# seorim0/DNN-based-Speech-Enhancement-in-the-frequency-domain

Measured on AMD Instinct MI355X. Metric: train utts/sec (3s@16kHz) DCCRN, higher is better.
Workload: dtype bf16; 1 GPU; DCCRN mask C, SI-SNR, fwd+bwd+Adam, B=32/GPU x 3s@16kHz clips (BASELINE configs[1]); global_batch=32, parallelism=dp1, bn=per-rank statistics, collective=none

## Files before the change

dnn-based-speech-enhancement-in-the-frequency-domain_amd/build.py:

```python
import os
import subprocess
from concurrent.futures import ThreadPoolExecutor

HERE = os.path.dirname(os.path.abspath(__file__))
CSRC = os.path.join(HERE, "csrc")
OBJ = os.path.join(CSRC, "_obj")
LIB = os.path.join(HERE, "libsefd_hip.so")
SOURCES = ["api.hip", "kernels.hip", "rungemm.hip", "rungemm_persist.hip", "cgemm256.hip", "enc0.hip", "lstm_bf16.hip", "lstm_cluster.hip", "lstm_rows.hip", "bn.hip", "cbn.hip", "lms.hip", "pmsqe.hip", "mix.hip", "composite.hip", "fsn.hip", "basemodel.hip", "stft_fft.hip", "thin.hip", "thin_mask.hip", "thin_stage.hip", "layout.hip", "optim.hip", "plan.cpp", "plan_dccrn.cpp", "plan_crn.cpp",
           "plan_fsn.cpp", "plan_seq.cpp", "plan_clstm.cpp", "plan_frontend.cpp", "plan_layers.cpp", "tuning.cpp"]


def _headers():
    hs = [os.path.join(CSRC, f) for f in os.listdir(CSRC) if f.endswith(".h")]
    hs.append(os.path.join(HERE, "..", "include", "sefd.h"))
    return [h for h in hs if os.path.exists(h)]


def _stale(target, deps):
    if not os.path.exists(target):
        return True
    t = os.path.getmtime(target)
    return any(os.path.getmtime(d) > t for d in deps)


def source_digest(paths, extra="") -> str:
    import hashlib
    h = hashlib.sha256(extra.encode())
    for p in sorted(paths):
        h.update(os.path.basename(p).encode())
        with open(p, "rb") as f:
            h.update(f.read())
    return h.hexdigest()


def stamp_current(lib, digest) -> bool:
    try:
        return os.path.exists(lib) and open(lib + ".stamp").read().strip() == digest
    except OSError:
        return False


def write_stamp(lib, digest):
    with open(lib + ".stamp", "w") as f:
        f.write(digest + "\n")


FLAGS = ["--offload-arch=gfx950", "-O3", "-std=c++17", "-fPIC"]


def _digest():
    return source_digest([os.path.join(CSRC, s) for s in SOURCES] + _headers(), " ".join(FLAGS + SOURCES))


def needs_build() -> bool:
    return not stamp_current(LIB, _digest())


def build(force: bool = False, verbose: bool = False) -> str:
    if not force and not needs_build():
        return LIB
    os.makedirs(OBJ, exist_ok=True)
    import fcntl
    with open(os.path.join(OBJ, ".build.lock"), "w") as lock:
        fcntl.flock(lock, fcntl.LOCK_EX)
        try:
            if not force and not needs_build():
                return LIB
            return _build_locked(force, verbose)
        finally:
            fcntl.flock(lock, fcntl.LOCK_UN)


def _build_locked(force, verbose) -> str:
    hipcc = os.environ.get("HIPCC", "/opt/rocm/bin/hipcc")
    heads = _headers()
    jobs = []
    for s in SOURCES:
        src, obj = os.path.join(CSRC, s), os.path.join(OBJ, s + ".o")
        if force or _stale(obj, [src] + heads):
            jobs.append([hipcc] + FLAGS + ["-c", "-o", obj, src])

    def run(cmd):
        if verbose:
            print(" ".join(cmd))
        subprocess.run(cmd, check=True, cwd=CSRC)

    with ThreadPoolExecutor(max_workers=int(os.environ.get("SEFD_BUILD_JOBS", "6"))) as ex:
        list(ex.map(run, jobs))
    run([hipcc, "--offload-arch=gfx950", "-fPIC", "-shared", "-o", LIB] + [os.path.join(OBJ, s + ".o") for s in SOURCES])
    write_stamp(LIB, _digest())
    return LIB


if __name__ == "__main__":
    print(build(force=True, verbose=True))
```

dnn-based-speech-enhancement-in-the-frequency-domain_amd/csrc/dev_common.h:

```cpp
#pragma once
#include <hip/hip_runtime.h>
#include "sefd_desc.h"

namespace sefd {

typedef __attribute__((ext_vector_type(4))) float f32x4;
typedef __attribute__((ext_vector_type(16))) float f32x16;
typedef __attribute__((ext_vector_type(8))) __bf16 bf16x8;

struct bf16_t { uint16_t v; };

struct ArenaBases { char* p[A_COUNT]; int* status; int* dstatus; };
__device__ __forceinline__ void set_status(int* host_word, int* dev_word) {
  if (host_word) __hip_atomic_store(host_word, 1, __ATOMIC_RELAXED, __HIP_MEMORY_SCOPE_SYSTEM);
  if (dev_word) __hip_atomic_store(dev_word, 1, __ATOMIC_RELAXED, __HIP_MEMORY_SCOPE_AGENT);
}

__host__ __device__ __forceinline__ char* rp(const ArenaBases& ab, const Ptr& q) { return ab.p[q.arena] + q.off; }

__device__ __forceinline__ uint32_t pack_bf16x2(float lo, float hi) {
  uint32_t r;
  asm("v_cvt_pk_bf16_f32 %0, %1, %2" : "=v"(r) : "v"(lo), "v"(hi));
  return r;
}
__device__ __forceinline__ uint16_t f2bf(float f) { return (uint16_t)pack_bf16x2(f, 0.f); }

struct QuadT {
  uint32_t sel;
  bool hi2;
  __device__ __forceinline__ explicit QuadT(int lane) : sel((lane & 1) ? 0x03020706u : 0x05040100u), hi2((lane & 2) != 0) {}
  __device__ __forceinline__ uint2 pack(uint32_t p01, uint32_t p23) const {
    const uint32_t n01 = (uint32_t)__builtin_amdgcn_mov_dpp((int)p01, 0xB1, 0xF, 0xF, true);
    const uint32_t n23 = (uint32_t)__builtin_amdgcn_mov_dpp((int)p23, 0xB1, 0xF, 0xF, true);
    const uint32_t q0 = __builtin_amdgcn_perm(n01, p01, sel);
    const uint32_t q1 = __builtin_amdgcn_perm(n23, p23, sel);
    const uint32_t send = hi2 ? q0 : q1, keep = hi2 ? q1 : q0;
    const uint32_t recv = (uint32_t)__builtin_amdgcn_mov_dpp((int)send, 0x4E, 0xF, 0xF, true);
    return make_uint2(hi2 ? recv : keep, hi2 ? keep : recv);
  }
  __device__ __forceinline__ uint2 pack(float v0, float v1, float v2, float v3) const { return pack(pack_bf16x2(v0, v1), pack_bf16x2(v2, v3)); }
};
__device__ __forceinline__ uint32_t xor4(uint32_t x, bool hi4) {
  const uint32_t up = (uint32_t)__builtin_amdgcn_update_dpp(0, (int)x, 0x104, 0xF, 0xF, true);
  const uint32_t dn = (uint32_t)__builtin_amdgcn_update_dpp(0, (int)x, 0x114, 0xF, 0xF, true);
  return hi4 ? dn : up;
}
struct OctW {
  bool hi4;
  __device__ __forceinline__ explicit OctW(int lane) : hi4((lane & 4) != 0) {}
  __device__ __forceinline__ void widen(const uint2 (&pk)[4], uint4 (&out)[2]) const {
#pragma unroll
    for (int h = 0; h < 2; ++h) {
      const uint2 keep = hi4 ? pk[2 * h + 1] : pk[2 * h], send = hi4 ? pk[2 * h] : pk[2 * h + 1];
      const uint2 recv = make_uint2(xor4(send.x, hi4), xor4(send.y, hi4));
      out[h] = hi4 ? make_uint4(recv.x, recv.y, keep.x, keep.y) : make_uint4(keep.x, keep.y, recv.x, recv.y);
    }
  }
};
__device__ __forceinline__ float bf2f(uint16_t h) { return __builtin_bit_cast(float, (uint32_t)h << 16); }

template <int DT> struct Elem;
__device__ __forceinline__ float ld_elem(const char* base, int dt, int64_t i) {
  return dt == DT_BF16 ? bf2f(reinterpret_cast<const uint16_t*>(base)[i]) : reinterpret_cast<const float*>(base)[i];
}
__device__ __forceinline__ void st_elem(char* base, int dt, int64_t i, float v) {
  if (dt == DT_BF16) reinterpret_cast<uint16_t*>(base)[i] = f2bf(v);
  else reinterpret_cast<float*>(base)[i] = v;
}

__device__ __forceinline__ float4 ld4(const char* base, int dt, int64_t i) {
  if (dt == DT_BF16) {
    const uint2 r = *reinterpret_cast<const uint2*>(base + i * 2);
    return make_float4(bf2f(r.x & 0xffff), bf2f(r.x >> 16), bf2f(r.y & 0xffff), bf2f(r.y >> 16));
  }
  return *reinterpret_cast<const float4*>(base + i * 4);
}
__device__ __forceinline__ void st4(char* base, int dt, int64_t i, float4 v) {
  if (dt == DT_BF16) {
    uint2 r;
    r.x = pack_bf16x2(v.x, v.y);
    r.y = pack_bf16x2(v.z, v.w);
    *reinterpret_cast<uint2*>(base + i * 2) = r;
  } else {
    *reinterpret_cast<float4*>(base + i * 4) = v;
  }
}

__device__ __forceinline__ void lds_barrier() {
  asm volatile("s_waitcnt lgkmcnt(0)\n\ts_barrier" ::: "memory");
}

__device__ __forceinline__ void dma16(const void* gsrc, uint32_t lds_wave_base) {
  asm volatile("s_mov_b32 m0, %0\n\ts_nop 0\n\tglobal_load_lds_dwordx4 %1, off" ::"s"(__builtin_amdgcn_readfirstlane(lds_wave_base)), "v"(gsrc)
               : "memory");
}
template <int N>
__device__ __forceinline__ void wait_vm() {
  asm volatile("s_waitcnt vmcnt(%0)" ::"n"(N) : "memory");
}
template <int NL, int S>
__device__ __forceinline__ void wait_stage(int rem) {
  if constexpr (S >= 4) { if (rem >= 2) { wait_vm<2 * NL>(); return; } }
  if constexpr (S >= 3) { if (rem >= 1) { wait_vm<NL>(); return; } }
  wait_vm<0>();
}
__device__ __forceinline__ uint32_t lds_addr(const void* p) {
  return (uint32_t)(uintptr_t)(__attribute__((address_space(3))) const void*)p;
}

__device__ __forceinline__ float wave_sum(float v) {
#pragma unroll
  for (int o = 32; o > 0; o >>= 1) v += __shfl_xor(v, o);
  return v;
}

__device__ __forceinline__ float sigmoidf_(float x) { return __builtin_amdgcn_rcpf(1.f + __expf(-x)); }
__device__ __forceinline__ float tanhf_(float x) { return 1.f - 2.f * __builtin_amdgcn_rcpf(__expf(2.f * x) + 1.f); }

__device__ __forceinline__ uint32_t mix32(uint32_t a, uint32_t b, uint32_t c) {
  uint32_t x = a * 0x9E3779B1u ^ (b + 0x7F4A7C15u) * 0x85EBCA77u ^ (c + 0x632BE5ABu) * 0xC2B2AE3Du;
  x ^= x >> 16; x *= 0x7FEB352Du; x ^= x >> 15; x *= 0x846CA68Bu; x ^= x >> 16;
  return x;
}
__device__ __forceinline__ float drop_scale(uint32_t seed0, uint32_t seed1, int layer, float keep, int64_t i) {
  if (keep >= 1.f) return 1.f;
  const uint32_t r = mix32(seed0 + (uint32_t)layer * 0x51ED27u, seed1 ^ (uint32_t)(i >> 32), (uint32_t)i);
  return ((r >> 8) * (1.f / 16777216.f)) < keep ? 1.f / keep : 0.f;
}

struct BnbCol { float mean, invstd, gamma, beta; };
__device__ __forceinline__ BnbCol bnb_col(const RunGemm& d, const ArenaBases& ab, int n) {
  BnbCol c{0.f, 0.f, 0.f, 0.f};
  if (n < d.N) {
    const float* mi = reinterpret_cast<const float*>(rp(ab, d.bnb_mi));
    c.mean = mi[n]; c.invstd = mi[d.N + n];
    c.gamma = reinterpret_cast<const float*>(rp(ab, d.bnb_gamma))[n];
    c.beta = reinterpret_cast<const float*>(rp(ab, d.bnb_beta))[n];
  }
  return c;
}
__device__ __forceinline__ void bnb_accum(const BnbCol& c, float slope, float dz, float yf, float& s0, float& s1, float& s2) {
  const float xh = (yf - c.mean) * c.invstd;
  const float bn = c.gamma * xh + c.beta;
  const float dbn = bn > 0.f ? dz : slope * dz;
  s0 += dbn;
  s1 += dbn * xh;
  s2 += bn > 0.f ? 0.f : bn * dz;
}

struct StreamKey {
  int dev; hipStream_t st;
  bool operator==(const StreamKey& o) const { return dev == o.dev && st == o.st; }
};
struct StreamKeyHash { size_t operator()(const StreamKey& k) const { return (size_t)(uintptr_t)k.st * 31u + (size_t)k.dev; } };
inline StreamKey stream_key(hipStream_t st) { int dev = 0; (void)hipGetDevice(&dev); return StreamKey{dev, st}; }

void launch_rungemm(const RunGemm& d, const ArenaBases& ab, hipStream_t st);
void launch_wgrad(const RunGemm& d, const ArenaBases& ab, hipStream_t st);
bool launch_cgemm256(const RunGemm& d, const ArenaBases& ab, hipStream_t st);
bool launch_enc0_fwd(const RunGemm& d, const ArenaBases& ab, hipStream_t st);
bool launch_enc0_wgrad(const RunGemm& d, const ArenaBases& ab, hipStream_t st);
bool launch_rundirect(const RunGemm& d, const ArenaBases& ab, hipStream_t st);
bool rundirect_takes(const RunGemm& d);
bool launch_rungemm_persist(const RunGemm& d, const ArenaBases& ab, hipStream_t st);
int rungemm_persist_grid(const RunGemm& d);
bool launch_thin_mask(const RunGemm& d, const ArenaBases& ab, hipStream_t st);
int thin_mask_grid(const RunGemm& d);
bool launch_thin_stage(const RunGemm& d, const ArenaBases& ab, hipStream_t st);
int thin_stage_grid(const RunGemm& d);
enum RunFamily : int { kFamNone = 0, kFamEnc0 = 1, kFamCgemm256 = 2, kFamDirect = 3, kFamTiled = 4, kFamPersist = 5, kFamThinMask = 6, kFamThinStage = 7 };
int rungemm_family(const RunGemm& d);
enum WgradFamily : int { kWgFamNone = 0, kWgFamEnc0 = 1, kWgFamEnc0Fused = 2, kWgFamRank = 3, kWgFamWide256 = 4, kWgFamWide256Ones = 5, kWgFamWide128 = 6,
                         kWgFamDma128 = 7, kWgFamDma64 = 8, kWgFamDma32 = 9, kWgFamBf16_128 = 10, kWgFamBf16_64 = 11, kWgFamF32 = 12 };
int wgrad_family(const RunGemm& d);
void launch_misc(const Op& op, const ArenaBases& ab, hipStream_t st);
void launch_stft_fft(const StftFft& d, const ArenaBases& ab, hipStream_t st);
void launch_istft_fft(const IstftFft& d, const ArenaBases& ab, hipStream_t st);
void launch_ifft_ola(const IfftOla& d, const ArenaBases& ab, hipStream_t st);
void launch_specconv(const SpecConv& d, const ArenaBases& ab, hipStream_t st);
void launch_ola_fold(const Ola& d, const ArenaBases& ab, hipStream_t st);
void launch_specout_adj(const SpecOut& d, const ArenaBases& ab, hipStream_t st);
void launch_nchw_cl(const NchwCl& d, const ArenaBases& ab, hipStream_t st);
void launch_fsn(const Op& op, const ArenaBases& ab, hipStream_t st);
void launch_bn(const Op& op, const ArenaBases& ab, hipStream_t st);
void launch_cbn(const Op& op, const ArenaBases& ab, hipStream_t st);
void launch_lstm_bf16(const LstmRec& d, const ArenaBases& ab, hipStream_t st, bool fwd);
inline int lstm_rev_groups(const LstmRec& d) { return d.rev_mask & ((1 << (d.G < 4 ? d.G : 4)) - 1); }
void launch_lstm_cluster(const LstmRec& d, const ArenaBases& ab, hipStream_t st, bool fwd);
void launch_lstm_rows(const LstmRec& d, const ArenaBases& ab, hipStream_t st, bool fwd);
bool launch_lstm_rows_pair(const LstmRec& d0, const LstmRec& d1, const ArenaBases& ab, hipStream_t st);

}
```

dnn-based-speech-enhancement-in-the-frequency-domain_amd/csrc/rungemm.hip:

```cpp
#include <hip/hip_runtime.h>
#include <cstdlib>
#include "sefd_desc.h"
#include "tuning.h"
#include "dev_common.h"

namespace sefd {

template <typename TA>
struct RowInfo {
  int64_t base0, base1;
  int32_t u, fo;
  bool valid;
};

template <typename TA>
__device__ __forceinline__ uint4 load_a_chunk(const RunGemm& d, const TA* x0, const TA* x1, const Seg& sg,
                                              int64_t base0, int64_t base1, int u, int fo, bool rvalid, int j0) {
  constexpr int VEC = 16 / sizeof(TA);
  uint4 z = make_uint4(0, 0, 0, 0);
  if (!rvalid) return z;
  if (sg.src < 0) {
    if (j0 == 0) {
      if (sizeof(TA) == 4) z.x = 0x3f800000u; else z.x = 0x3f80u;
    }
// ... 1053 lines not shown
#pragma unroll
    for (int e = 0; e < 8; ++e) acc[n][e] = 0.f;
  }
  auto row = [&](const uint4 xv, const float (&g)[NR]) {
    const uint32_t w[4] = {xv.x, xv.y, xv.z, xv.w};
#pragma unroll
    for (int e = 0; e < 8; ++e) {
      const float xe = bf2f((uint16_t)(w[e >> 1] >> (16 * (e & 1))));
#pragma unroll
      for (int n = 0; n < NR; ++n) acc[n][e] = fmaf(g[n], xe, acc[n][e]);
    }
#pragma unroll
    for (int n = 0; n < NR; ++n) bs[n] += g[n];
  };
  auto ldy = [&](int64_t m, float (&g)[NR]) {
#pragma unroll
    for (int n = 0; n < NR; ++n) g[n] = n < d.N ? bf2f(dy[m * ys + n]) : 0.f;
  };
  if (act) {
    int64_t m = m0 + rl;
    for (; m + 3 * RL < m1; m += 4 * RL) {
      uint4 xv[4];
      float g[4][NR];
#pragma unroll
      for (int u = 0; u < 4; ++u) { xv[u] = *reinterpret_cast<const uint4*>(x + (m + u * RL) * fs); ldy(m + u * RL, g[u]); }
#pragma unroll
      for (int u = 0; u < 4; ++u) row(xv[u], g[u]);
    }
    for (; m < m1; m += RL) {
      float g[NR];
      ldy(m, g);
      row(*reinterpret_cast<const uint4*>(x + m * fs), g);
    }
#pragma unroll
    for (int n = 0; n < NR; ++n) {
#pragma unroll
      for (int e = 0; e < 8; ++e) red[(rl * NR + n) * K + 8 * kc + e] = acc[n][e];
      if (kc == 0) redb[rl][n] = bs[n];
    }
  }
  for (int i = tid; i < d.Npad * d.ldw; i += 256) part[i] = 0.f;
  __syncthreads();
  for (int i = tid; i < d.N * K; i += 256) {
    const int n = i / K, k = i - n * K;
    float v = red[n * K + k];
    for (int r = 1; r < RL; ++r) v += red[(r * NR + n) * K + k];
    part[(int64_t)n * d.ldw + sg.koff + k] = v;
  }
  if (d.nseg == 2 && tid < d.N) {
    float v = redb[0][tid];
    for (int r = 1; r < RL; ++r) v += redb[r][tid];
    part[(int64_t)tid * d.ldw + d.seg[1].koff] = v;
  }
}

static bool launch_wgrad_rank(const RunGemm& d, const ArenaBases& ab, hipStream_t st) {
  if (!(d.flags & kRunRank) || !wgrad_rank_form(d)) return false;
  const dim3 grid((unsigned)d.nsplit);
  if (d.N <= 2) hipLaunchKernelGGL((wgrad_rank_kernel<2>), grid, dim3(256), 0, st, d, ab);
  else hipLaunchKernelGGL((wgrad_rank_kernel<4>), grid, dim3(256), 0, st, d, ab);
  return true;
}

template <typename TA, int BN>
static void launch_rungemm_dma(const RunGemm& d, const ArenaBases& ab, hipStream_t st, int grid) {
  if (d.flags & kRunBnBwd) { hipLaunchKernelGGL((rungemm_kernel<TA, BN, true, 2, kBM, 4, false, true>), dim3(grid), dim3(256), 0, st, d, ab); return; }
  hipLaunchKernelGGL((rungemm_kernel<TA, BN, true, 2>), dim3(grid), dim3(256), 0, st, d, ab);
}

template <typename TA>
static void launch_rungemm_t(const RunGemm& d, const ArenaBases& ab, hipStream_t st) {
  const int bn = bn_of(d.N);
  const int nm = (d.M + kBM - 1) / kBM;
  const int grid = nm * (d.Npad / bn);
  if constexpr (sizeof(TA) == 2) {
    if (launch_rungemm_persist(d, ab, st)) return;
  }
  if (d.flags & kRunAligned) {
    if (bn == 128) launch_rungemm_dma<TA, 128>(d, ab, st, grid);
    else if (bn == 64) launch_rungemm_dma<TA, 64>(d, ab, st, grid);
    else launch_rungemm_dma<TA, 32>(d, ab, st, grid);
    return;
  }
  if (d.flags & kRunBnBwd) {
    if (bn == 128) hipLaunchKernelGGL((rungemm_kernel<TA, 128, false, 2, kBM, 4, false, true>), dim3(grid), dim3(256), 0, st, d, ab);
    else if (bn == 64) hipLaunchKernelGGL((rungemm_kernel<TA, 64, false, 2, kBM, 4, false, true>), dim3(grid), dim3(256), 0, st, d, ab);
    else hipLaunchKernelGGL((rungemm_kernel<TA, 32, false, 2, kBM, 4, false, true>), dim3(grid), dim3(256), 0, st, d, ab);
    return;
  }
  if (bn == 128) hipLaunchKernelGGL((rungemm_kernel<TA, 128, false>), dim3(grid), dim3(256), 0, st, d, ab);
  else if (bn == 64) hipLaunchKernelGGL((rungemm_kernel<TA, 64, false>), dim3(grid), dim3(256), 0, st, d, ab);
  else hipLaunchKernelGGL((rungemm_kernel<TA, 32, false>), dim3(grid), dim3(256), 0, st, d, ab);
}

__global__ void refuse_launch_kernel(int* host_word, int* dev_word) { set_status(host_word, dev_word); }

static void refuse_launch(const ArenaBases& ab, hipStream_t st) {
  hipLaunchKernelGGL(refuse_launch_kernel, dim3(1), dim3(1), 0, st, ab.status, ab.dstatus);
}

void launch_rungemm(const RunGemm& d, const ArenaBases& ab, hipStream_t st) {
  if (launch_enc0_fwd(d, ab, st)) return;
  if (d.flags & (kRunEnc0 | kRunDyFromBn)) { refuse_launch(ab, st); return; }
  if (launch_cgemm256(d, ab, st)) return;
  if (launch_thin_mask(d, ab, st)) return;
  if (launch_thin_stage(d, ab, st)) return;
  if (launch_rundirect(d, ab, st)) return;
  if (d.xdt == DT_BF16) launch_rungemm_t<bf16_t>(d, ab, st);
  else launch_rungemm_t<float>(d, ab, st);
}

int rungemm_family(const RunGemm& d) {
  if ((d.flags & kRunEnc0) && enc0_accepts(d, false)) return kFamEnc0;
  if (d.flags & (kRunEnc0 | kRunDyFromBn)) return kFamNone;
  if (d.flags & kRunWTile32) return kFamCgemm256;
  if (thin_mask_grid(d) > 0) return kFamThinMask;
  if (thin_stage_grid(d) > 0) return kFamThinStage;
  if (rundirect_takes(d)) return kFamDirect;
  if (d.xdt == DT_BF16 && rungemm_persist_grid(d) > 0) return kFamPersist;
  return kFamTiled;
}

static void launch_wgrad_wide(const RunGemm& d, const ArenaBases& ab, hipStream_t st) {
  if (d.flags & kRunOnesMfma) {
    dim3 grid1(((d.Npad + 255) / 256) * ((d.ldw - 64 + 255) / 256) * d.nsplit);
    hipLaunchKernelGGL((wgrad_bf16_dma_kernel<256, 4, 256, 512, true, true>), grid1, dim3(512), 0, st, d, ab);
    return;
  }
  dim3 grid(((d.Npad + 255) / 256) * ((d.ldw + 255) / 256) * d.nsplit);
  hipLaunchKernelGGL((wgrad_bf16_dma_kernel<256, 4, 256, 512, true>), grid, dim3(512), 0, st, d, ab);
}

static void launch_wgrad_wide128(const RunGemm& d, const ArenaBases& ab, hipStream_t st) {
  dim3 grid(((d.Npad + 127) / 128) * ((d.ldw + 511) / 512) * d.nsplit);
  hipLaunchKernelGGL((wgrad_bf16_dma_kernel<128, 2, 512, 512>), grid, dim3(512), 0, st, d, ab);
}

template <int TN>
static void launch_wgrad_dma(const RunGemm& d, const ArenaBases& ab, hipStream_t st) {
  dim3 grid(((d.Npad + TN - 1) / TN) * ((d.ldw + kWgTK - 1) / kWgTK) * d.nsplit);
  hipLaunchKernelGGL((wgrad_bf16_dma_kernel<TN, 3>), grid, dim3(256), 0, st, d, ab);
}

void launch_wgrad(const RunGemm& d0, const ArenaBases& ab, hipStream_t st) {
  if (launch_enc0_wgrad(d0, ab, st)) return;
  if (d0.flags & (kRunEnc0 | kRunDyFromBn)) { refuse_launch(ab, st); return; }
  if (launch_wgrad_rank(d0, ab, st)) return;
  RunGemm d = d0;
#ifdef SEFD_TUNING
  if (tune_int("WG_DBG", 0) & 8) d.flags |= 1 << 30;
#endif
  if (d.xdt == DT_BF16 && (d.flags & kRunAligned)) {
    if (d.flags & kRunWgWide) { if (d.Npad % 256 == 0) launch_wgrad_wide(d, ab, st); else launch_wgrad_wide128(d, ab, st); return; }
    switch (wgrad_tn(d.xdt, d.N, d.Npad)) {
      case 128: launch_wgrad_dma<128>(d, ab, st); break;
      case 64: launch_wgrad_dma<64>(d, ab, st); break;
      default: launch_wgrad_dma<32>(d, ab, st); break;
    }
    return;
  }
  if (d.xdt == DT_BF16) {
    if (d.Npad >= 128) {
      dim3 grid(((d.Npad + 127) / 128) * ((d.ldw + kWgTK - 1) / kWgTK) * d.nsplit);
      hipLaunchKernelGGL((wgrad_bf16_kernel<128>), grid, dim3(256), 0, st, d, ab);
    } else {
      dim3 grid(((d.Npad + 63) / 64) * ((d.ldw + kWgTK - 1) / kWgTK) * d.nsplit);
      hipLaunchKernelGGL((wgrad_bf16_kernel<64>), grid, dim3(256), 0, st, d, ab);
    }
    return;
  }
  dim3 grid(((d.Npad + kWgTN - 1) / kWgTN) * ((d.ldw + kWgTK - 1) / kWgTK) * d.nsplit);
  hipLaunchKernelGGL((wgrad_kernel<float>), grid, dim3(256), 0, st, d, ab);
}

int wgrad_family(const RunGemm& d) {
  if ((d.flags & kRunEnc0) && enc0_accepts(d, true)) return (d.flags & kRunDyFromBn) ? kWgFamEnc0Fused : kWgFamEnc0;
  if (d.flags & (kRunEnc0 | kRunDyFromBn)) return kWgFamNone;
  if ((d.flags & kRunRank) && wgrad_rank_form(d)) return kWgFamRank;
  if (d.xdt == DT_BF16 && (d.flags & kRunAligned)) {
    if (d.flags & kRunWgWide) return d.Npad % 256 != 0 ? kWgFamWide128 : (d.flags & kRunOnesMfma) ? kWgFamWide256Ones : kWgFamWide256;
    switch (wgrad_tn(d.xdt, d.N, d.Npad)) {
      case 128: return kWgFamDma128;
      case 64: return kWgFamDma64;
      default: return kWgFamDma32;
    }
  }
  if (d.xdt == DT_BF16) return d.Npad >= 128 ? kWgFamBf16_128 : kWgFamBf16_64;
  return kWgFamF32;
}

}
```

dnn-based-speech-enhancement-in-the-frequency-domain_amd/plan.py:

```python
import ctypes as C
from collections import OrderedDict

import numpy as np
import torch

from . import _lib

ARENA_WS, ARENA_PARAM, ARENA_GRAD, ARENA_STATE, ARENA_CONST, ARENA_IO, ARENA_COUNT = 0, 1, 2, 3, 4, 5, 6
PHASE_FWD, PHASE_BWD = 0, 1
RUN_FAMILY_NONE, RUN_FAMILY_ENC0, RUN_FAMILY_CGEMM256, RUN_FAMILY_DIRECT, RUN_FAMILY_TILED, RUN_FAMILY_PERSIST, RUN_FAMILY_THIN_MASK, RUN_FAMILY_THIN_STAGE = range(8)
(WG_FAMILY_NONE, WG_FAMILY_ENC0, WG_FAMILY_ENC0_FUSED, WG_FAMILY_RANK, WG_FAMILY_WIDE256, WG_FAMILY_WIDE256_ONES, WG_FAMILY_WIDE128,
 WG_FAMILY_DMA128, WG_FAMILY_DMA64, WG_FAMILY_DMA32, WG_FAMILY_BF16_128, WG_FAMILY_BF16_64, WG_FAMILY_F32) = range(13)
WG_FAMILY_NAMES = ("none", "first layer", "first layer fused", "rank-N", "256 x 256", "256 x 256 ones MFMA", "128 x 512", "aligned 128", "aligned 64",
                   "aligned 32", "unaligned bf16 128", "unaligned bf16 64", "fp32")
RUN_WAVE_ONLY = 1
MASK_MODES = {"E": 0, "C": 1, "R": 2, "Direct(None make)": 4}
DTYPES = {"fp32": 0, "float32": 0, "bf16": 1, "bfloat16": 1}


CONV_KINDS = {"ComplexConv2d": 0, "ComplexConvTranspose2d": 1, "RealConv2d": 2, "RealConvTranspose2d": 3}
FSN_NORMS = {"offline_laplace_norm": 0, "cumulative_laplace_norm": 1, "offline_gaussian_norm": 2, "cumulative_layer_norm": 3}


class Plan:
    def __init__(self, B, L, kernel_num=(32, 64, 128, 256, 256, 256), rnn_layers=2, rnn_units=256, win_len=400,
                 win_inc=100, fft_len=512, masking_mode="E", lstm="complex", skip_type=True, act_dtype="fp32",
                 kernel_size=5, training=True, model="DCCRN", fsn=None, bn_world=1, grad_buckets=1, use_cbn=False, win_type="hanning",
                 cbn_sync=False, seq=None, feature_type="complex", conv=None, cbn=None, clstm=None):
        self.lib = _lib.lib()
        if masking_mode not in MASK_MODES:
            raise NotImplementedError(f"masking_mode {masking_mode!r} is not on the HIP path yet")
        cfg = _lib.ModelConfig()
        cfg.model = {"DCCRN": 0, "CRN": 1, "STFT": 2, "FullSubNet": 3, "TorchSTFT": 4, "TorchISTFT": 5, "SequenceModel": 6, "ConvSTFT": 7,
                     "ConviSTFT": 8, "ConvLayer": 9, "ComplexBatchNorm": 10, "ComplexLSTM": 11, "TorchSTFTAdj": 12, "TorchISTFTAdj": 13}[model]
        cfg.B, cfg.L = int(B), int(L)
        if model == "FullSubNet":
            f = dict(sb_num_neighbors=15, fb_num_neighbors=0, look_ahead=2, fb_hidden=512, sb_hidden=384, fb_act="ReLU",
                     sb_act=None, keep=0.2, sequence_model="LSTM", norm_type="offline_laplace_norm")
            f.update(fsn or {})
            acts = {None: 0, "None": 0, "ReLU": 1, "Tanh": 2, "ReLU6": 3}
            kernel_num = (f["sb_num_neighbors"], f["fb_num_neighbors"], f["look_ahead"], f["fb_hidden"], f["sb_hidden"],
                          acts[f["fb_act"]], acts[f["sb_act"]], int(round(f["keep"] * 1000)),
                          {"LSTM": 0, "GRU": 1}[f["sequence_model"]], FSN_NORMS[f["norm_type"]])
        if model == "SequenceModel":
            s = dict(input_size=257, output_size=257, hidden_size=512, num_layers=2, bidirectional=False, sequence_model="LSTM", keep=0.2)
            s.update(seq or {})
            if s["sequence_model"] not in ("LSTM", "GRU"):
                raise NotImplementedError(f"Not implemented {s['sequence_model']}")
            kernel_num = (s["input_size"], s["output_size"], s["hidden_size"], s["num_layers"], 1 if s["bidirectional"] else 0,
                          {"LSTM": 0, "GRU": 1}[s["sequence_model"]], int(round(s["keep"] * 1000)))
            self.seq = s
        if model in ("ConvSTFT", "ConviSTFT"):
            kernel_num = (0 if feature_type == "complex" else 1,)
        if model == "ConvLayer":
            v = dict(kind="ComplexConv2d", in_channels=2, out_channels=2, kernel_size=(1, 1), stride_f=1, padding=(0, 0), causal=True, output_padding_f=0, F=1)
            v.update(conv or {})
            kernel_num = (CONV_KINDS[v["kind"]], v["in_channels"], v["out_channels"], v["kernel_size"][0], v["kernel_size"][1], v["stride_f"],
                          v["padding"][0], v["padding"][1], 1 if v["causal"] else 0, v["output_padding_f"], v["F"])
            self.conv = v
        if model == "ComplexBatchNorm":
            v = dict(num_features=8, eps=1e-5, momentum=0.1)
            v.update(cbn or {})
            bits = lambda f: int(np.float32(f).view(np.int32))
            kernel_num = (v["num_features"], bits(v["eps"]), bits(v["momentum"]))
            self.cbn = v
        if model == "ComplexLSTM":
            v = dict(input_size=2, hidden_size=16, projection_dim=None, bidirectional=False)
            v.update(clstm or {})
            for k in ("input_size", "hidden_size", "projection_dim"):
                if v[k] is not None and v[k] % 2:
                    raise ValueError(f"sefd plan: ComplexLSTM: {k} {v[k]} is odd: it has no real / imaginary halves")
            if v["projection_dim"] is not None and v["projection_dim"] < 2:
                raise ValueError(f"sefd plan: ComplexLSTM: projection_dim / 2 must be at least 1, got projection_dim {v['projection_dim']} (None: no projection)")
            kernel_num = (v["input_size"] // 2, v["hidden_size"] // 2, 0 if v["projection_dim"] is None else v["projection_dim"] // 2, 1 if v["bidirectional"] else 0)
            self.clstm = v
        cfg.win_len, cfg.hop, cfg.fft_len = win_len, win_inc, fft_len
        cfg.n_layers = len(kernel_num) if model not in ("FullSubNet", "SequenceModel", "ConvSTFT", "ConviSTFT", "ConvLayer", "ComplexBatchNorm", "ComplexLSTM") else 0
        for i, k in enumerate(kernel_num):
            cfg.kernel_num[i] = int(k)
        cfg.rnn_layers, cfg.rnn_units = rnn_layers, rnn_units
        cfg.mask_mode = MASK_MODES[masking_mode]
        cfg.lstm_complex = 1 if lstm == "complex" else 0
        cfg.skip = 1 if skip_type else 0
        cfg.act_dtype = DTYPES[act_dtype]
        cfg.kernel_size = kernel_size
        cfg.training = 1 if training else 0
        cfg.bn_world = int(bn_world)
        cfg.grad_buckets = int(grad_buckets)
        cfg.use_cbn = 1 if use_cbn else 0
        cfg.cbn_sync = 1 if cbn_sync else 0
        if win_type in (None, "None"):
            cfg.window = 1
        elif win_type in ("hanning", "hann"):
            cfg.window = 0
        else:
            from .frontend_consts import window_fn
            self._window_values = np.ascontiguousarray(window_fn(win_type, win_len), dtype=np.float64)
            cfg.window = 2
            cfg.window_values = self._window_values.ctypes.data_as(C.POINTER(C.c_double))
        self.cfg = cfg
        self.model_name = model
        self.masking_mode = masking_mode
        self.h = self.lib.sefd_plan_create(C.byref(cfg))
        err = self.lib.sefd_plan_error(self.h).decode()
        if err:
            self.lib.sefd_plan_destroy(self.h)
            self.h = None
            raise ValueError("sefd plan: " + err)
        self.B, self.L = int(B), int(L)
        self.T = self.lib.sefd_plan_frames(self.h)
        self.NF = fft_len // 2 + 1
        self.arena_bytes = [self.lib.sefd_plan_arena_bytes(self.h, a) for a in range(ARENA_COUNT)]
        self.params = self._param_table(0)
        self.state = self._param_table(1)
        self.n_param = sum(int(np.prod(s)) if len(s) else 1 for _, s in self.params.values()) if self.params else 0
        self.n_state = sum(int(np.prod(s)) if len(s) else 1 for _, s in self.state.values())

    def sync_points(self):
        out = []
        ph, op, ar, dt = C.c_int32(), C.c_int32(), C.c_int32(), C.c_int32()
        off, cnt = C.c_int64(), C.c_int64()
        for i in range(self.lib.sefd_plan_num_syncs(self.h)):
            self.lib.sefd_plan_sync(self.h, i, C.byref(ph), C.byref(op), C.byref(ar), C.byref(off), C.byref(cnt), C.byref(dt))
            out.append((ph.value, op.value, ar.value, off.value, cnt.value, torch.float64 if dt.value else torch.float32))
        return out

    def run_synced(self, phase, arenas, stream, all_reduce):
        cur = 0
        for ph, op, ar, off, cnt, dtype in self.sync_points():
            if ph != phase:
                continue
            self.run(phase, arenas, stream, cur, op + 1)
            nbytes = cnt * (8 if dtype == torch.float64 else 4)
            all_reduce(arenas[ar].view(torch.uint8)[off:off + nbytes].view(dtype))
            cur = op + 1
        self.run(phase, arenas, stream, cur, self.num_ops(phase))

    def _param_table(self, kind):
        out = OrderedDict()
        shp = (C.c_int64 * 4)()
        for i in range(self.lib.sefd_plan_num_params(self.h, kind)):
            name = self.lib.sefd_plan_param_name(self.h, kind, i).decode()
            nd = self.lib.sefd_plan_param_shape(self.h, kind, i, shp)
            out[name] = (self.lib.sefd_plan_param_offset(self.h, kind, i), tuple(int(shp[k]) for k in range(nd)))
        return out

    def __del__(self):
        if getattr(self, "h", None):
            self.lib.sefd_plan_destroy(self.h)
            self.h = None

    def num_ops(self, phase):
        return self.lib.sefd_plan_num_ops(self.h, phase)

    def ops_ptr(self, phase):
        return self.lib.sefd_plan_ops(self.h, phase)

    def op_kinds(self, phase):
        n, sz = self.num_ops(phase), self.lib.sefd_op_size()
        raw = np.ctypeslib.as_array((C.c_int32 * (n * sz // 4)).from_address(self.ops_ptr(phase))).reshape(n, sz // 4)
        return raw[:, 0].copy(), raw[:, 1].copy()

    def op_info(self, phase, i):
        o = (C.c_int64 * 8)()
        if self.lib.sefd_plan_op_info(self.h, phase, i, o) != 0:
            raise IndexError(i)
        return dict(kind=int(o[0]), tag=int(o[1]), M=int(o[2]), N=int(o[3]), K=int(o[4]), dtype=int(o[5]) & 0xff, flags=(int(o[5]) >> 8) & 0xffffffff,
# ... 102 lines not shown
```

Measured before the change: 3195 utt/s.

## Add frame-staged thin weight-gradient kernel for narrow-channel conv layers

Adds a specialized wgrad kernel for bf16 conv layers with 8/16/32 input channels and 32/64 outputs. It stages each input frame and its output-gradient frame into LDS through a multi-slot async DMA ring, reuses adjacent frames across the two time taps, and feeds MFMA using transposed LDS reads. It replaces the generic aligned DMA wgrad for large-M cases. The cost is a new code path with strict shape and stride checks, plus per-split partial sums that still have to be reduced.

```diff
diff --git a/dnn-based-speech-enhancement-in-the-frequency-domain_amd/build.py b/dnn-based-speech-enhancement-in-the-frequency-domain_amd/build.py
--- a/dnn-based-speech-enhancement-in-the-frequency-domain_amd/build.py
+++ b/dnn-based-speech-enhancement-in-the-frequency-domain_amd/build.py
@@ -6,7 +6,7 @@
 CSRC = os.path.join(HERE, "csrc")
 OBJ = os.path.join(CSRC, "_obj")
 LIB = os.path.join(HERE, "libsefd_hip.so")
-SOURCES = ["api.hip", "kernels.hip", "rungemm.hip", "rungemm_persist.hip", "cgemm256.hip", "enc0.hip", "lstm_bf16.hip", "lstm_cluster.hip", "lstm_rows.hip", "bn.hip", "cbn.hip", "lms.hip", "pmsqe.hip", "mix.hip", "composite.hip", "fsn.hip", "basemodel.hip", "stft_fft.hip", "thin.hip", "thin_mask.hip", "thin_stage.hip", "layout.hip", "optim.hip", "plan.cpp", "plan_dccrn.cpp", "plan_crn.cpp",
+SOURCES = ["api.hip", "kernels.hip", "rungemm.hip", "rungemm_persist.hip", "cgemm256.hip", "enc0.hip", "lstm_bf16.hip", "lstm_cluster.hip", "lstm_rows.hip", "bn.hip", "cbn.hip", "lms.hip", "pmsqe.hip", "mix.hip", "composite.hip", "fsn.hip", "basemodel.hip", "stft_fft.hip", "thin.hip", "thin_mask.hip", "thin_stage.hip", "thin_wgrad.hip", "layout.hip", "optim.hip", "plan.cpp", "plan_dccrn.cpp", "plan_crn.cpp",
            "plan_fsn.cpp", "plan_seq.cpp", "plan_clstm.cpp", "plan_frontend.cpp", "plan_layers.cpp", "tuning.cpp"]
 
 
diff --git a/dnn-based-speech-enhancement-in-the-frequency-domain_amd/csrc/dev_common.h b/dnn-based-speech-enhancement-in-the-frequency-domain_amd/csrc/dev_common.h
--- a/dnn-based-speech-enhancement-in-the-frequency-domain_amd/csrc/dev_common.h
+++ b/dnn-based-speech-enhancement-in-the-frequency-domain_amd/csrc/dev_common.h
@@ -171,8 +171,10 @@
 enum RunFamily : int { kFamNone = 0, kFamEnc0 = 1, kFamCgemm256 = 2, kFamDirect = 3, kFamTiled = 4, kFamPersist = 5, kFamThinMask = 6, kFamThinStage = 7 };
 int rungemm_family(const RunGemm& d);
 enum WgradFamily : int { kWgFamNone = 0, kWgFamEnc0 = 1, kWgFamEnc0Fused = 2, kWgFamRank = 3, kWgFamWide256 = 4, kWgFamWide256Ones = 5, kWgFamWide128 = 6,
-                         kWgFamDma128 = 7, kWgFamDma64 = 8, kWgFamDma32 = 9, kWgFamBf16_128 = 10, kWgFamBf16_64 = 11, kWgFamF32 = 12 };
+                         kWgFamDma128 = 7, kWgFamDma64 = 8, kWgFamDma32 = 9, kWgFamBf16_128 = 10, kWgFamBf16_64 = 11, kWgFamF32 = 12, kWgFamThin = 13 };
 int wgrad_family(const RunGemm& d);
+bool launch_thin_wgrad(const RunGemm& d, const ArenaBases& ab, hipStream_t st);
+bool thin_wgrad_takes(const RunGemm& d);
 void launch_misc(const Op& op, const ArenaBases& ab, hipStream_t st);
 void launch_stft_fft(const StftFft& d, const ArenaBases& ab, hipStream_t st);
 void launch_istft_fft(const IstftFft& d, const ArenaBases& ab, hipStream_t st);
diff --git a/dnn-based-speech-enhancement-in-the-frequency-domain_amd/csrc/rungemm.hip b/dnn-based-speech-enhancement-in-the-frequency-domain_amd/csrc/rungemm.hip
--- a/dnn-based-speech-enhancement-in-the-frequency-domain_amd/csrc/rungemm.hip
+++ b/dnn-based-speech-enhancement-in-the-frequency-domain_amd/csrc/rungemm.hip
@@ -1229,6 +1229,7 @@
 #endif
   if (d.xdt == DT_BF16 && (d.flags & kRunAligned)) {
     if (d.flags & kRunWgWide) { if (d.Npad % 256 == 0) launch_wgrad_wide(d, ab, st); else launch_wgrad_wide128(d, ab, st); return; }
+    if (launch_thin_wgrad(d0, ab, st)) return;
     switch (wgrad_tn(d.xdt, d.N, d.Npad)) {
       case 128: launch_wgrad_dma<128>(d, ab, st); break;
       case 64: launch_wgrad_dma<64>(d, ab, st); break;
@@ -1256,6 +1257,7 @@
   if ((d.flags & kRunRank) && wgrad_rank_form(d)) return kWgFamRank;
   if (d.xdt == DT_BF16 && (d.flags & kRunAligned)) {
     if (d.flags & kRunWgWide) return d.Npad % 256 != 0 ? kWgFamWide128 : (d.flags & kRunOnesMfma) ? kWgFamWide256Ones : kWgFamWide256;
+    if (thin_wgrad_takes(d)) return kWgFamThin;
     switch (wgrad_tn(d.xdt, d.N, d.Npad)) {
       case 128: return kWgFamDma128;
       case 64: return kWgFamDma64;
diff --git a/dnn-based-speech-enhancement-in-the-frequency-domain_amd/csrc/thin_wgrad.hip b/dnn-based-speech-enhancement-in-the-frequency-domain_amd/csrc/thin_wgrad.hip
--- /dev/null
+++ b/dnn-based-speech-enhancement-in-the-frequency-domain_amd/csrc/thin_wgrad.hip
@@ -0,0 +1,246 @@
+#include <hip/hip_runtime.h>
+#include <cstdlib>
+#include "sefd_desc.h"
+#include "tuning.h"
+#include "dev_common.h"
+
+namespace sefd {
+
+namespace {
+
+constexpr int64_t kThinWgradMinRows = 262144;
+
+typedef __attribute__((ext_vector_type(4))) short s16x4;
+struct Frag8 { s16x4 lo, hi; };
+
+template <int CRUN, int N>
+struct WgGeom {
+  static constexpr int FO = CRUN == 8 ? 128 : 64;
+  static constexpr int SPF = FO / kWgRows;
+  static constexpr int CPT = CRUN / 8;
+  static constexpr int RPB = CRUN * 2;
+  static constexpr int PLANE = (FO + 2) * RPB;
+  static constexpr int RUNB = 2 * PLANE;
+  static constexpr int DCH = N / 8;
+  static constexpr int DPB = N * 2;
+  static constexpr int SLOT = RUNB + FO * DPB;
+  static constexpr int SEGLEN = 5 * CRUN;
+  static constexpr int SEGPAD = (SEGLEN + 63) / 64 * 64;
+  static constexpr int LDW = 2 * SEGPAD;
+  static constexpr int KBS = (SEGLEN + 15) / 16;
+  static constexpr int PADC = SEGPAD - 16 * KBS;
+  static constexpr int WPS = N == 64 ? 2 : 1;
+  static constexpr int NWN = 4 / (2 * WPS);
+  static constexpr int NT = N / 16 / NWN;
+  static constexpr int KB = KBS / WPS;
+  static constexpr int NIT_R = 2 * FO * CPT / 256;
+  static constexpr int NIT_D = FO * DCH / 256;
+  static constexpr int NI = NIT_R + NIT_D;
+  static constexpr int S = CRUN == 32 ? 5 : CRUN == 16 ? 4 : 3;
+  static_assert((N == 64 || N == 32) && (CRUN == 32 || CRUN == 16 || CRUN == 8) && KBS % WPS == 0 && NIT_R >= 1 && NIT_D >= 1 && NT >= 1, "instantiated forms");
+  static_assert((FO * CPT) % 64 == 0 && (FO * DCH) % 64 == 0, "a wave's 64 chunks stay inside one plane");
+  __host__ __device__ static constexpr int swz_run(int row) { return CPT == 4 ? ((row >> 2) & 1) << 1 : 0; }
+  __host__ __device__ static constexpr int swz_den(int pos) { return DCH == 8 ? ((pos >> 1) & 3) << 1 : ((pos >> 2) & 1) << 1; }
+};
+
+__device__ __forceinline__ bf16x8 tr_pair(const char* smem, int lo, int hi) {
+  Frag8 f;
+  f.lo = __builtin_amdgcn_ds_read_tr16_b64_v4i16((__attribute__((address_space(3))) s16x4*)(smem + lo));
+  f.hi = __builtin_amdgcn_ds_read_tr16_b64_v4i16((__attribute__((address_space(3))) s16x4*)(smem + hi));
+  return __builtin_bit_cast(bf16x8, f);
+}
+
+}
+
+template <int CRUN, int N>
+__global__ __launch_bounds__(256) void thin_wgrad_kernel(const RunGemm d, const ArenaBases ab) {
+  using G = WgGeom<CRUN, N>;
+  constexpr int FO = G::FO, SPF = G::SPF, CPT = G::CPT, RPB = G::RPB, PLANE = G::PLANE, RUNB = G::RUNB, DCH = G::DCH, DPB = G::DPB, SLOT = G::SLOT;
+  constexpr int NT = G::NT, KB = G::KB, NIT_R = G::NIT_R, NIT_D = G::NIT_D, NI = G::NI, S = G::S, LDW = G::LDW;
+  __shared__ __attribute__((aligned(16))) char smem[S * SLOT];
+  const int tid = threadIdx.x, lane = tid & 63, wid = __builtin_amdgcn_readfirstlane(tid >> 6);
+  const int li = lane & 15, q = lane >> 4;
+  const int split = blockIdx.x;
+  float* part = reinterpret_cast<float*>(rp(ab, d.w)) + (int64_t)split * N * LDW;
+
+  const int Tout = d.Tout, Tin = d.Tin[0];
+  const int spb = Tout * SPF;
+  const int nsteps_total = (int)(d.M / ((int64_t)Tout * FO)) * spb;
+  const int per = (nsteps_total + d.nsplit - 1) / d.nsplit;
+  const int64_t s0 = (int64_t)split * per;
+  const int step0 = (int)(s0 < nsteps_total ? s0 : nsteps_total);
+  const int step1 = nsteps_total < step0 + per ? nsteps_total : step0 + per;
+
+  const int wn = wid % G::NWN, wk = wid / G::NWN;
+  const int sg = wk / G::WPS, blk0 = (wk % G::WPS) * KB;
+  const int kcol0 = d.seg[sg].koff + 16 * blk0;
+
+  f32x4 acc[NT][KB];
+#pragma unroll
+  for (int a = 0; a < NT; ++a)
+#pragma unroll
+    for (int b = 0; b < KB; ++b) acc[a][b] = f32x4{0.f, 0.f, 0.f, 0.f};
+
+  if (step0 < step1) {
+    const uint16_t* x0 = reinterpret_cast<const uint16_t*>(rp(ab, d.x[0]));
+    const uint16_t* dy = reinterpret_cast<const uint16_t*>(rp(ab, d.y));
+    const uint16_t* zp = reinterpret_cast<const uint16_t*>(rp(ab, d.zero));
+    const int hi = d.seg[0].dt > d.seg[1].dt ? d.seg[0].dt : d.seg[1].dt;
+    const bool lo_run = d.seg[sg].dt != hi;
+
+    const int r0 = 4 * q + (li >> 2), c4 = 4 * (li & 3);
+    int doff[NT][2], koff[KB][2], kstep[KB];
+#pragma unroll
+    for (int a = 0; a < NT; ++a)
+#pragma unroll
+      for (int h = 0; h < 2; ++h) {
+        const int pos = r0 + 16 * h, col = 16 * (wn * NT + a) + c4;
+        doff[a][h] = RUNB + pos * DPB + (((col >> 3) ^ G::swz_den(pos)) << 4) + (col & 7) * 2;
+      }
+#pragma unroll
+    for (int b = 0; b < KB; ++b)
+#pragma unroll
+      for (int h = 0; h < 2; ++h) {
+        const int j = 16 * (blk0 + b) + c4;
+        const int tap = j / CRUN, ch = j % CRUN;
+        const int row = r0 + 16 * h + (tap >> 1);
+        const bool data = 16 * G::KBS == G::SEGLEN || j < G::SEGLEN;
+        koff[b][h] = data ? (tap & 1) * PLANE + row * RPB + (((ch >> 3) ^ G::swz_run(row)) << 4) + (ch & 7) * 2 : 0;
+        kstep[b] = data ? kWgRows * RPB : 0;
+      }
+
+    int roff[NIT_R], rdst[NIT_R], yoff[NIT_D], ydst[NIT_D];
+#pragma unroll
+    for (int it = 0; it < NIT_R; ++it) {
+      const int L = it * 256 + tid, plane = L / (FO * CPT), within = L % (FO * CPT), row = 1 + within / CPT, c = (within % CPT) ^ G::swz_run(row);
+      roff[it] = (2 * (row - 1) + plane) * CRUN + c * 8;
+      const int L0 = it * 256 + wid * 64;
+      rdst[it] = (L0 / (FO * CPT)) * PLANE + RPB + (L0 % (FO * CPT)) * 16;
+    }
+#pragma unroll
+    for (int it = 0; it < NIT_D; ++it) {
+      const int L = it * 256 + tid, pos = L / DCH, c = (L % DCH) ^ G::swz_den(pos);
+      yoff[it] = pos * d.y_fstride + c * 8;
+      ydst[it] = RUNB + (it * 256 + wid * 64) * 16;
+    }
+    const uint32_t lbase = lds_addr(smem);
+    const int64_t bs0 = d.bstride[0], ybs = d.y_bstride;
+    const int ts0 = d.tstride[0], ba0 = d.base[0], yts = d.y_tstride, yo = d.y_off;
+
+    const int b0 = step0 / spb, u0 = (step0 - b0 * spb) / SPF;
+    const int b1 = (step1 - 1) / spb, u1 = (step1 - 1 - b1 * spb) / SPF;
+    const int nv = (b1 - b0) * (Tout + 1) + u1 - u0 + 2;
+    int ib = b0, iu = u0 - 1, iv = 0, islot = 0;
+    auto issue = [&]() {
+      const bool in = iv < nv;
+      const int t = iu + hi;
+      const bool rv = in && t >= 0 && t < Tin, dv = in && iu >= 0 && iv > 0;
+      const uint16_t* fr = x0 + (int64_t)ib * bs0 + ba0 + (int64_t)t * ts0;
+      const uint16_t* fd = dy + (int64_t)ib * ybs + (int64_t)iu * yts + yo;
+      const uint32_t sl = lbase + islot * SLOT;
+#pragma unroll
+      for (int it = 0; it < NIT_R; ++it) dma16(rv ? fr + roff[it] : zp, sl + rdst[it]);
+#pragma unroll
+      for (int it = 0; it < NIT_D; ++it) dma16(dv ? fd + yoff[it] : zp, sl + ydst[it]);
+      ++iv;
+      if (++iu == Tout) { iu = -1; ++ib; }
+      islot = islot + 1 == S ? 0 : islot + 1;
+    };
+    for (int i = tid; i < S * 4 * CPT; i += 256) {
+      const int r = i / CPT, slot = r / 4, plane = (r >> 1) & 1, last = r & 1;
+      *reinterpret_cast<uint4*>(smem + slot * SLOT + plane * PLANE + (last ? (FO + 1) * RPB : 0) + (i % CPT) * 16) = make_uint4(0, 0, 0, 0);
+    }
+#pragma unroll
+    for (int i = 0; i < S - 2; ++i) issue();
+
+    int cb = b0, cu = u0 - 1, cur = 0, prev = (S - 1) * SLOT;
+    for (int v = 0; v < nv; ++v) {
+      wait_vm<(S - 3) * NI>();
+      lds_barrier();
+      issue();
+      if (cu >= 0) {
+        const int sbase = cb * spb + cu * SPF;
+        const int rslot = lo_run ? prev : cur;
+#pragma unroll
+        for (int h = 0; h < SPF; ++h) {
+          const int s = sbase + h;
+          if (s >= step0 && s < step1) {
+            bf16x8 af[NT], bfr[KB];
+#pragma unroll
+            for (int a = 0; a < NT; ++a) af[a] = tr_pair(smem, cur + doff[a][0] + h * kWgRows * DPB, cur + doff[a][1] + h * kWgRows * DPB);
+#pragma unroll
+            for (int b = 0; b < KB; ++b) bfr[b] = tr_pair(smem, rslot + koff[b][0] + h * kstep[b], rslot + koff[b][1] + h * kstep[b]);
+#pragma unroll
+            for (int a = 0; a < NT; ++a)
+#pragma unroll
+              for (int b = 0; b < KB; ++b) acc[a][b] = __builtin_amdgcn_mfma_f32_16x16x32_bf16(af[a], bfr[b], acc[a][b], 0, 0, 0);
+          }
+        }
+      }
+      if (++cu == Tout) { cu = -1; ++cb; }
+      prev = cur;
+      cur = cur + SLOT == S * SLOT ? 0 : cur + SLOT;
+    }
+    wait_vm<0>();
+  }
+
+#pragma unroll
+  for (int a = 0; a < NT; ++a)
+#pragma unroll
+    for (int b = 0; b < KB; ++b)
+#pragma unroll
+      for (int r = 0; r < 4; ++r) {
+        const int n = 16 * (wn * NT + a) + 4 * q + r;
+        part[(int64_t)n * LDW + kcol0 + 16 * b + li] = acc[a][b][r];
+      }
+  if constexpr (G::PADC > 0) {
+    for (int i = tid; i < N * 2 * G::PADC; i += 256) {
+      const int n = i / (2 * G::PADC), c = i % (2 * G::PADC), s = c / G::PADC;
+      part[(int64_t)n * LDW + d.seg[s].koff + 16 * G::KBS + c % G::PADC] = 0.f;
+    }
+  }
+}
+
+namespace {
+
+int wgrad_thin_form(const RunGemm& d) {
+  if (d.xdt != DT_BF16 || d.ydt != DT_BF16 || !(d.flags & kRunAligned)) return 0;
+  if (d.flags & ~(kRunAligned | kRunYAligned)) return 0;
+  if (d.zero.arena < 0 || d.x[0].arena < 0 || d.x[1].arena >= 0 || d.y.arena < 0 || d.w.arena < 0 || d.nseg != 2 || d.nsplit < 1) return 0;
+  if (d.fstride[0] % 2 != 0 || d.N != d.Npad) return 0;
+  const int C = d.fstride[0] / 2, N = d.N;
+  if (!((C == 32 && N == 64) || (C == 16 && N == 32) || (C == 8 && N == 32))) return 0;
+  const int Fo = C == 8 ? 128 : 64;
+  if (d.Fo != Fo || d.Tout <= 0 || d.M <= 0 || (int64_t)d.M % ((int64_t)d.Tout * Fo) != 0 || d.Tin[0] <= 0) return 0;
+  if (d.rowlen[0] != 2 * Fo * C || d.tstride[0] % 8 != 0 || d.base[0] % 8 != 0 || d.bstride[0] % 8 != 0 || d.x[0].off % 16 != 0) return 0;
+  if (d.y_fstride % 8 != 0 || d.y_fstride < N || d.y_off % 8 != 0 || d.y_tstride % 8 != 0 || d.y_bstride % 8 != 0 || d.y.off % 16 != 0) return 0;
+  const int hi = d.seg[0].dt > d.seg[1].dt ? d.seg[0].dt : d.seg[1].dt, lo = d.seg[0].dt < d.seg[1].dt ? d.seg[0].dt : d.seg[1].dt;
+  if (lo != hi - 1) return 0;
+  const int pad = (5 * C + 63) / 64 * 64;
+  for (int s = 0; s < 2; ++s)
+    if (d.seg[s].src != 0 || d.seg[s].off != -2 * C || d.seg[s].len != 5 * C || d.seg[s].koff != s * pad) return 0;
+  if (d.ldw != 2 * pad) return 0;
+  return C + 256 * N;
+}
+
+}
+
+bool thin_wgrad_takes(const RunGemm& d) {
+  const int mode = (int)tune_int("THIN_WGRAD", 1);
+  if (mode <= 0) return false;
+  if (!wgrad_thin_form(d)) return false;
+  return mode == 2 || d.M >= kThinWgradMinRows;
+}
+
+bool launch_thin_wgrad(const RunGemm& d, const ArenaBases& ab, hipStream_t st) {
+  if (!thin_wgrad_takes(d)) return false;
+  const dim3 grid((unsigned)d.nsplit);
+  switch (wgrad_thin_form(d)) {
+    case 32 + 256 * 64: hipLaunchKernelGGL((thin_wgrad_kernel<32, 64>), grid, dim3(256), 0, st, d, ab); break;
+    case 16 + 256 * 32: hipLaunchKernelGGL((thin_wgrad_kernel<16, 32>), grid, dim3(256), 0, st, d, ab); break;
+    default: hipLaunchKernelGGL((thin_wgrad_kernel<8, 32>), grid, dim3(256), 0, st, d, ab); break;
+  }
+  return true;
+}
+
+}
diff --git a/dnn-based-speech-enhancement-in-the-frequency-domain_amd/plan.py b/dnn-based-speech-enhancement-in-the-frequency-domain_amd/plan.py
--- a/dnn-based-speech-enhancement-in-the-frequency-domain_amd/plan.py
+++ b/dnn-based-speech-enhancement-in-the-frequency-domain_amd/plan.py
@@ -10,9 +10,14 @@
 PHASE_FWD, PHASE_BWD = 0, 1
 RUN_FAMILY_NONE, RUN_FAMILY_ENC0, RUN_FAMILY_CGEMM256, RUN_FAMILY_DIRECT, RUN_FAMILY_TILED, RUN_FAMILY_PERSIST, RUN_FAMILY_THIN_MASK, RUN_FAMILY_THIN_STAGE = range(8)
 (WG_FAMILY_NONE, WG_FAMILY_ENC0, WG_FAMILY_ENC0_FUSED, WG_FAMILY_RANK, WG_FAMILY_WIDE256, WG_FAMILY_WIDE256_ONES, WG_FAMILY_WIDE128,
- WG_FAMILY_DMA128, WG_FAMILY_DMA64, WG_FAMILY_DMA32, WG_FAMILY_BF16_128, WG_FAMILY_BF16_64, WG_FAMILY_F32) = range(13)
+ WG_FAMILY_DMA128, WG_FAMILY_DMA64, WG_FAMILY_DMA32, WG_FAMILY_BF16_128, WG_FAMILY_BF16_64, WG_FAMILY_F32, WG_FAMILY_THIN) = range(14)
 WG_FAMILY_NAMES = ("none", "first layer", "first layer fused", "rank-N", "256 x 256", "256 x 256 ones MFMA", "128 x 512", "aligned 128", "aligned 64",
                    "aligned 32", "unaligned bf16 128", "unaligned bf16 64", "fp32")
+WG_FAMILY_MORE_NAMES = {WG_FAMILY_THIN: "frame-staged thin"}
+
+
+def wg_family_name(family):
+    return WG_FAMILY_MORE_NAMES[family] if family in WG_FAMILY_MORE_NAMES else WG_FAMILY_NAMES[family]
 RUN_WAVE_ONLY = 1
 MASK_MODES = {"E": 0, "C": 1, "R": 2, "Direct(None make)": 4}
 DTYPES = {"fp32": 0, "float32": 0, "bf16": 1, "bfloat16": 1}
```

Result: faster. 3268 utt/s (median of 6 runs) (+2.3%).
